# url-kaist/UV-SLAM

Hardware: AMD Instinct MI355X
Metric: sliding-window solves/sec (10 KF, 150 pts, 40 lines, 3 VP) (higher is better)
Workload: dtype f64; 1 GPU; W10-P150-L40-V3 x 256 independent windows per GPU (BASELINE configs[2]); single window (configs[1]) in single_window, the 20k-point window (configs[3]) in large_window (both with --full); windows_per_gpu=256, frames=11, points=150, lines=40, vp_tagged_lines=30, prior=True, parallelism=replicas x1

## Files before the change

### uv-slam_amd/csrc/uvs_solve_kernel.h

```cpp
#pragma once
#include <hip/hip_runtime.h>
#include <initializer_list>
#include <utility>
#include "../../include/uvs_solver.h"
#include "uvs_layout.h"
#include "uvs_factors.h"

namespace uvsdev {

#ifndef UVS_UNIT
#define UVS_UNIT unit
#endif

#ifndef UVS_X_PLAIN_TID
static __device__ __forceinline__ int lane_tid() { int t = threadIdx.x; asm volatile("" : "+v"(t)); return t; }
#else
static __device__ __forceinline__ int lane_tid() { return threadIdx.x; }
#endif
static constexpr int NT = UVS_NT;
static constexpr int NW = NT / 64;
static constexpr bool ROLES = NT > 256;
static constexpr int ET = ROLES ? 256 : NT;
static constexpr int EW = ET / 64;
static constexpr int GT0 = NT - UVS_GT;
// ... 14 lines not shown
static_assert(UVS_PT_C == UVS_PT_A + 12, "pt_anchor_pass reads A and c as one run");
static constexpr int CP_PB = NT > 256 ? UVS_T_CP_PB : 4;
static constexpr int CP_LB = NT > 256 ? UVS_T_CP_LB : 2;
static constexpr int BS_LNB = NT > 256 ? UVS_T_BS_LNB : 4;
static constexpr int PR_UN = NT > 256 ? UVS_T_PR_UN : 26;
static constexpr int PG_UN = NT > 256 ? 16 : 32;

static constexpr int L_X = 0;
static constexpr int L_XC = L_X + UVS_XDIM;
static constexpr int L_G = L_XC + UVS_XDIM;
static constexpr int L_DLT = L_G + UVS_RD;
static constexpr int L_HD = L_DLT + UVS_RD + 24;
static constexpr int L_SC = L_HD + UVS_RD;
static constexpr int L_DD = L_SC + UVS_RD;
static constexpr int L_DINV = L_DD + UVS_RD;
static constexpr int L_RF = L_DINV + UVS_RD;
static constexpr int L_EX = L_RF + 120;
static constexpr int L_PDX = L_EX + 16;
static constexpr int L_PR = L_PDX + UVS_MAX_PRIOR_DIM;
static constexpr int L_PRC = L_PR + UVS_MAX_PRIOR_DIM;
static constexpr int L_RED = L_PRC + UVS_MAX_PRIOR_DIM;
static constexpr int L_CTRL = L_RED + (5 * NW > 24 ? 5 * NW : 24);
static constexpr int L_PROF = L_CTRL + 32;
static constexpr int L_WPROF = L_PROF + 24;
static constexpr int L_LCOST = L_WPROF + 8;
static constexpr int LACC = 1;
static constexpr int L_LGMAX = L_LCOST + ET / LACC;
static constexpr int L_PX0 = L_LGMAX + 8;
static constexpr int L_PTAB = L_PX0 + 9 * UVS_MAX_PRIOR_BLOCKS;
static constexpr int L_SMALL = (L_PTAB + 2 * UVS_MAX_PRIOR_BLOCKS + 1) & ~1;
static constexpr int L_S = L_SMALL;
static constexpr int L_TOTAL = L_S + UVS_S_DOUBLES;
static_assert(L_TOTAL * 8 <= 160 * 1024, "LDS map exceeds the 160 KB of a CU");
enum { P_SETUP = 0, P_OBS, P_LMPREP, P_GATHER, P_ASSEMBLE, P_CHOL, P_TRSV, P_BACKSUB, P_COST, P_MISC, P_CH_DIAG, P_CH_PANEL, P_CH_TRAIL, P_AS_IMU, P_AS_ZERO, P_AS_ADD, P_LAST };
#define UVS_PROF(c, k) do { if ((c).o.debug && lane_tid() == 0) { const long long now_ = clock64(); (c).sh[L_PROF + (k)] += (double)(now_ - (long long)(c).sh[L_PROF + 23]); (c).sh[L_PROF + 23] = (double)now_; } } while (0)
static constexpr size_t LDS_BYTES = (size_t)L_TOTAL * 8;
static constexpr int TL_PER_WAVE = 4096;
inline namespace UVS_UNIT { __device__ long long g_lin_tl[8 * TL_PER_WAVE * 2]; }
#define UVS_TLOG(c, id) do { if ((c).o.debug == 5 && (threadIdx.x & 63) == 0 && blockIdx.x == 0) { const int w_ = threadIdx.x >> 6; const int n_ = (int)(c).sh[L_WPROF + w_]; \
    if (n_ < TL_PER_WAVE) { g_lin_tl[2 * (w_ * TL_PER_WAVE + n_)] = (id); g_lin_tl[2 * (w_ * TL_PER_WAVE + n_) + 1] = clock64(); (c).sh[L_WPROF + w_] = (double)(n_ + 1); } } } while (0)

enum { C_COST = 0, C_RADIUS, C_DECR, C_XNORM, C_GMAX, C_CAND, C_MCC, C_STEP2, C_XC2, C_GO, C_IT, C_INVALID, C_CUR, C_FIRST,
       C_TERM, C_NSUCC, C_CHOLOK, C_GMAXLM, C_TIMEUP };

struct KOpts {
    int max_it, ex_free, keep_cand, jacobi;
    double sqrt_info, line_factor, vp_factor, loss_pt, loss_ln, loss_vp, G[3];
    double r0, rmax, rmin, min_rel, dlo, dhi, ftol, gtol, ptol;
    int max_invalid;
    int debug;
    long long max_ticks;
    int redamp;
    int line_ahead;
};

inline namespace UVS_UNIT {
__constant__ unsigned char c_blk_fa[UVS_NBLK];
__constant__ unsigned char c_blk_fb[UVS_NBLK];
}

UVS_DEV int sidx(int i, int j) {
    const int bi = i >> 4, bj = j >> 4;
    return (((bi * (bi + 1)) >> 1) + bj) * UVS_BLK_SZ + (i & 15) * UVS_BLK_LD + (j & 15);
}
UVS_DEV double bcast_lane(double v, int lane) {
    const int lo = __builtin_amdgcn_readlane(__double2loint(v), lane);
    const int hi = __builtin_amdgcn_readlane(__double2hiint(v), lane);
    return __hiloint2double(hi, lo);
}
UVS_DEV void wave_sync() {
    __builtin_amdgcn_fence(__ATOMIC_RELEASE, "wavefront");
    __builtin_amdgcn_wave_barrier();
    __builtin_amdgcn_fence(__ATOMIC_ACQUIRE, "wavefront");
}

UVS_DEV double wave_sum(double v) {
#pragma unroll
    for (int off = 32; off > 0; off >>= 1) v += __shfl_down(v, off, 64);
    return v;
}
UVS_DEV double wave_max(double v) {
#pragma unroll
    for (int off = 32; off > 0; off >>= 1) v = fmax(v, __shfl_down(v, off, 64));
    return v;
}
UVS_DEV void rsqrt_pair(double x, double* sq, double* rsq) {
    const double y = __builtin_amdgcn_rsq(x);
    double g = x * y, hh = 0.5 * y;
    double r = fma(-hh, g, 0.5);
    g = fma(g, r, g); hh = fma(hh, r, hh);
    r = fma(-hh, g, 0.5);
    g = fma(g, r, g); hh = fma(hh, r, hh);
    const double d = fma(-g, g, x);
    g = fma(d, hh, g);
    *sq = g; *rsq = 2.0 * hh;
}
UVS_DEV void block_reduce(double* sh, double* s , double* mx) {
    const int tid = lane_tid(), lane = tid & 63, wv = tid >> 6;
    __syncthreads();
#pragma unroll
    for (int k = 0; k < 4; ++k) { const double t = wave_sum(s[k]); if (lane == 0) sh[L_RED + wv * 5 + k] = t; }
    { const double t = wave_max(*mx); if (lane == 0) sh[L_RED + wv * 5 + 4] = t; }
    __syncthreads();
    double a[4] = {0, 0, 0, 0}, m = 0.0;
#pragma unroll
    for (int w = 0; w < NW; ++w) {
// ... 1123 lines not shown
    UVS_TLOG(c, 43);
}
UVS_DEV double lin_imu_tiles(const Ctx& c, ImuN& N) {
    DevWinK& h = *c.hdr;
    double* sh = c.sh;
    const int tid = lane_tid(), lane = tid & 63, wv = UVS_KWAVE(tid), li = lane & 15, lk = lane >> 4;
    double cost = 0.0;
    double* IM = sh + L_S;
    IntK* itab = (IntK*)c.bi + h.i_imu;
    bool act[IMU_SLOTS];
#pragma unroll
    for (int s = 0; s < IMU_SLOTS; ++s) {
        const int b = imu_block_of(wv, s);
        act[s] = b < h.n_imu && !itab[2 * (b < h.n_imu ? b : 0) + 1];
        N.act[s] = act[s]; N.fi[s] = itab[2 * (b < h.n_imu ? b : 0)];
        if (act[s]) {
            double* Jb = IM + IMU_BLK * b; const double* Wb = Jb + IMU_WOFF;
            d4_t t0 = {0.0, 0.0, 0.0, 0.0}, t1 = t0;
            double wa[4], j0[4], j1[4];
#pragma unroll
            for (int q = 0; q < 4; ++q) { wa[q] = Wb[li * UVS_BLK_LD + 4 * q + lk]; j0[q] = Jb[(4 * q + lk) * IMU_JLD + li]; j1[q] = Jb[(4 * q + lk) * IMU_JLD + 16 + li]; }
#pragma unroll
            for (int q = 0; q < 4; ++q) { t0 = __builtin_amdgcn_mfma_f64_16x16x4f64(wa[q], j0[q], t0, 0, 0, 0); t1 = __builtin_amdgcn_mfma_f64_16x16x4f64(wa[q], j1[q], t1, 0, 0, 0); }
#pragma unroll
            for (int q = 0; q < 4; ++q) { Jb[(lk + 4 * q) * IMU_JLD + li] = t0[q]; Jb[(lk + 4 * q) * IMU_JLD + 16 + li] = t1[q]; }
        }
    }
    wave_sync();
#pragma unroll
    for (int s = 0; s < IMU_SLOTS; ++s) {
        const int b = imu_block_of(wv, s);
        d4_t n00 = {0.0, 0.0, 0.0, 0.0}, n10 = n00, n11 = n00;
        if (act[s]) {
            const double* Jb = IM + IMU_BLK * b;
            double j0[4], j1[4];
#pragma unroll
            for (int q = 0; q < 4; ++q) { j0[q] = Jb[(4 * q + lk) * IMU_JLD + li]; j1[q] = Jb[(4 * q + lk) * IMU_JLD + 16 + li]; }
#pragma unroll
            for (int q = 0; q < 4; ++q) {
                n00 = __builtin_amdgcn_mfma_f64_16x16x4f64(j0[q], j0[q], n00, 0, 0, 0);
                n10 = __builtin_amdgcn_mfma_f64_16x16x4f64(j1[q], j0[q], n10, 0, 0, 0);
                n11 = __builtin_amdgcn_mfma_f64_16x16x4f64(j1[q], j1[q], n11, 0, 0, 0);
            }
            if (lane == 63) cost += 0.5 * n11[3];
        }
        N.n00[s] = n00; N.n10[s] = n10; N.n11[s] = n11;
    }
    UVS_PROF(c, P_AS_IMU);
    return cost;
}
UVS_DEV double lin_imu(const Ctx& c, const double* x, ImuN& N) { lin_imu_stage(c, x); return lin_imu_tiles(c, N); }
UVS_DEV double lin_frames(const Ctx& c, const double* x, ImuN& N) { const double pc = lin_prep(c, x); return pc + lin_imu(c, x, N); }

UVS_DEV void spd4_inverse(const double* H, const double* gl, double* X, double* hg) {
    double L[10];
    double i0, i1, i2, i3;
    rsqrt_pair(H[0], &L[0], &i0);
    L[1] = H[1] * i0; rsqrt_pair(H[2] - L[1] * L[1], &L[2], &i1);
    L[3] = H[3] * i0; L[4] = (H[4] - L[3] * L[1]) * i1; rsqrt_pair(H[5] - L[3] * L[3] - L[4] * L[4], &L[5], &i2);
    L[6] = H[6] * i0; L[7] = (H[7] - L[6] * L[1]) * i1; L[8] = (H[8] - L[6] * L[3] - L[7] * L[4]) * i2;
    rsqrt_pair(H[9] - L[6] * L[6] - L[7] * L[7] - L[8] * L[8], &L[9], &i3);
    hg[0] = 0.0; hg[1] = 0.0; hg[2] = 0.0; hg[3] = 0.0;
#pragma unroll
    for (int cidx = 0; cidx < 4; ++cidx) {
        double e[4] = {0, 0, 0, 0}; e[cidx] = 1.0;
        e[0] = e[0] * i0;
        e[1] = (e[1] - L[1] * e[0]) * i1;
        e[2] = (e[2] - L[3] * e[0] - L[4] * e[1]) * i2;
        e[3] = (e[3] - L[6] * e[0] - L[7] * e[1] - L[8] * e[2]) * i3;
        e[3] = e[3] * i3;
        e[2] = (e[2] - L[8] * e[3]) * i2;
        e[1] = (e[1] - L[4] * e[2] - L[7] * e[3]) * i1;
        e[0] = (e[0] - L[1] * e[1] - L[3] * e[2] - L[6] * e[3]) * i0;
        X[0 * 4 + cidx] = e[0]; X[1 * 4 + cidx] = e[1]; X[2 * 4 + cidx] = e[2]; X[3 * 4 + cidx] = e[3];
#pragma unroll
        for (int a = 0; a < 4; ++a) hg[a] += e[a] * gl[cidx];
    }
}

#ifndef UVS_X_NO_LISTS_BY_GATHERERS
static constexpr bool LISTS_BY_GATHERERS = ROLES;
#else
static constexpr bool LISTS_BY_GATHERERS = false;
#endif
struct ChunkDesc { int type, k0, k1, o0, nob, nlm, nlist; const int* glists; };
UVS_DEV ChunkDesc chunk_desc(const Ctx& c, int ch) {
    DevWinK& h = *c.hdr;
    IntK* chunks = (IntK*)c.bi + h.i_chunks + UVS_CHUNK_INTS * UVS_KIDX(ch);
    ChunkDesc d;
    d.type = chunks[0]; d.k0 = chunks[1]; d.k1 = chunks[2];
    d.glists = c.bi + h.i_lists + chunks[3];
    d.nlist = chunks[4];
    d.nlm = d.k1 - d.k0;
    d.o0 = chunks[6]; d.nob = chunks[7];
    return d;
}
UVS_DEV int* chunk_lists(const Ctx& c, const ChunkDesc& d) {
    DevWinK& h = *c.hdr;
    double* rec = c.sh + L_S;
    if (d.type == 0) return (int*)(rec + (size_t)d.nob * h.pt_rec + (size_t)(d.nob + h.pt_xslots * d.nlm) * 12);
    return (int*)(rec + (size_t)d.nob * (UVS_LN_REC + 2 * UVS_LN_EY) + 20 * d.nlm);
}
UVS_DEV void pt_landmark_slots(const Ctx& c, const ChunkDesc& d, int k, int b0, int b1, double hd, double gl, double dd, double hinv, double ginv, double* gmax_lm) {
    DevWinK& h = *c.hdr;
    const int PREC = h.pt_rec, XS = h.pt_xslots, li = k - d.k0;
    double* rec = c.sh + L_S;
    double* Eb = rec + (size_t)d.nob * PREC;
    double* EIb = Eb + (size_t)(d.nob + XS * d.nlm) * 6;
    double* E = Eb + (size_t)(b0 + XS * li) * 6; double* EI = EIb + (size_t)(b0 + XS * li) * 6;
    double* Eg = c.ws + h.w_pt_E + 6 * (size_t)(d.o0 + b0 + XS * k);
        double* px = c.ws + h.w_pt_x + 4 * (size_t)k; px[0] = ginv; px[1] = gl; px[2] = dd; px[3] = hd;
        *gmax_lm = fmax(*gmax_lm, fabs(gl));
        double e0[6] = {0, 0, 0, 0, 0, 0}, etd = 0.0;
        for (int o = b0; o < b1; ++o) {
            const double* Ro = rec + (size_t)o * PREC;
#pragma unroll
            for (int a = 0; a < 6; ++a) e0[a] += Ro[UVS_PT_C] * Ro[UVS_PT_A + a] + Ro[UVS_PT_C + 1] * Ro[UVS_PT_A + 6 + a];
            if (h.td_on) etd += Ro[UVS_PT_C] * Ro[UVS_PT_TD] + Ro[UVS_PT_C + 1] * Ro[UVS_PT_TD + 1];
        }
#pragma unroll
        for (int a = 0; a < 6; ++a) { E[a] = e0[a]; EI[a] = e0[a] * hinv; Eg[a] = e0[a] * hinv; }
        if (h.td_on) {
            const int st_ = 6 * (b1 - b0 + 1);
#pragma unroll
            for (int a = 0; a < 6; ++a) { const double e = a == 0 ? etd : 0.0; E[st_ + a] = e; EI[st_ + a] = e * hinv; Eg[st_ + a] = e * hinv; }
        }
        if (h.ex_on) {
            double ex6[6] = {0, 0, 0, 0, 0, 0};
            for (int o = b0; o < b1; ++o) {
                const double* Ro = rec + (size_t)o * PREC;
// ... 79 lines not shown
        double* Eb = c.sh + L_S + (size_t)d.nob * PREC;
        double* E = Eb + (size_t)(b0 + li) * 6; double* EI = E + (size_t)(d.nob + d.nlm) * 6;
#pragma unroll
        for (int a = 0; a < 6; ++a) { E[a] = e0[a]; EI[a] = e0[a] * hinv; Eg[a] = e0[a] * hinv; }
    }
    lacc_add(c.sh, 0.0, gmax_lm);
}
UVS_DEV void chunk_touch(const Ctx& c, const ChunkDesc& d, const double* invd, const double* line) {
    DevWinK& h = *c.hdr;
    const int tid = lane_tid();
    if (tid >= d.nob) return;
    const int o = d.o0 + tid;
    double acc = 0.0; int iacc = 0;
    if (d.type == 0) {
        const int lm = c.bi[h.i_pt_lm + o]; iacc = c.bi[h.i_pt_fi + o] + c.bi[h.i_pt_fj + o];
        const double* m = c.bd + h.d_ptmeas + o; const int st = h.pt_stride;
#pragma unroll
        for (int q = 0; q < 6; ++q) acc += m[q * st];
        acc += invd[lm] + c.ws[h.w_scale_pt + lm];
        iacc += c.bi[h.i_pt_beg + lm] + c.bi[h.i_pt_beg + lm + 1];
    } else {
        const int lm = c.bi[h.i_ln_lm + o]; iacc = c.bi[h.i_ln_fj + o] + c.bi[h.i_ln_vp + o];
#ifndef UVS_X_NO_TOUCH_B1
        iacc += c.bi[h.i_ln_beg + lm] + c.bi[h.i_ln_beg + lm + 1];
        acc += c.ws[h.w_scale_ln + 4 * lm] + c.ws[h.w_scale_ln + 4 * lm + 3];
#endif
        const double* m = c.bd + h.d_lnmeas + o; const int st = h.ln_stride;
#pragma unroll
        for (int q = 0; q < 9; ++q) acc += m[q * st];
        const double* ltrig = line_trig_of(c, line);
        if (ltrig) {
#pragma unroll
            for (int q = 0; q < 8; ++q) acc += ltrig[8 * lm + q];
        } else {
#pragma unroll
            for (int q = 0; q < 4; ++q) acc += line[4 * lm + q];
        }
    }
    asm volatile("" :: "v"(acc), "v"(iacc));
}
static constexpr int LG_UN = 16;
UVS_DEV void copy_lists_gatherers(const Ctx& c, const ChunkDesc& d) {
    int* lists = chunk_lists(c, d);
    const int t0 = lane_tid() - GT0;
    for (int tb = t0; tb < d.nlist; tb += LG_UN * UVS_GT) {
        int w[LG_UN];
#pragma unroll
        for (int u = 0; u < LG_UN; ++u) { const int t = tb + u * UVS_GT; w[u] = d.glists[t < d.nlist ? t : tb]; }
#pragma unroll
        for (int u = 0; u < LG_UN; ++u) { const int t = tb + u * UVS_GT; if (t < d.nlist) lists[t] = w[u]; }
    }
}
UVS_DEV double line_pass_a(const Ctx& c, const ChunkDesc& d, const double* x, const double* line, int rec_base);
UVS_DEV void line_pass_b(const Ctx& c, const ChunkDesc& d, bool first, double radius, double cost, int rec_base);
UVS_DEV void chunk_eval(const Ctx& c, const ChunkDesc& d, const double* x, const double* invd, const double* line, bool first, double radius) {
    DevWinK& h = *c.hdr;
    double* sh = c.sh;
    const int tid = lane_tid();
    const double* RF = sh + L_RF; const double* ric = sh + L_EX; const double* tic = sh + L_EX + 9;
    double cost = 0.0, gmax_lm = 0.0;
    {
        const int type = d.type, k0 = d.k0, k1 = d.k1;
        const int* glists = d.glists;
        const int nlist = d.nlist;
        const int nlm = d.nlm;
        UVS_TLOG(c, 1);
        __syncthreads();
        UVS_PROF(c, P_GATHER);
        UVS_TLOG(c, 2);
        if (type == 0) {
            const int* beg = c.bi + h.i_pt_beg;
            const int o0 = d.o0, nob = d.nob, o1 = o0 + nob;
            const int PREC = h.pt_rec, XS = h.pt_xslots;
            double* rec = sh + L_S;
            double* Eb = rec + (size_t)nob * PREC;
            double* EIb = Eb + (size_t)(nob + XS * nlm) * 6;
            int* lists = (int*)(EIb + (size_t)(nob + XS * nlm) * 6);
            if (!LISTS_BY_GATHERERS) for (int t = tid; t < nlist; t += ET) lists[t] = glists[t];
            for (int o = o0 + tid; o < o1; o += ET) {
                const int lm = c.bi[h.i_pt_lm + o], fi = c.bi[h.i_pt_fi + o], fj = c.bi[h.i_pt_fj + o];
                double pi[3], pj[3], vij[4] = {0.0, 0.0, 0.0, 0.0};
                load_point_obs(c, o, x[183], pi, pj, vij);
                double r[2], A[12], B[12], cl[2], jtd[2] = {0.0, 0.0};
                point_eval<true, false>(x + 7 * fi, RF + 9 * fi, pose_of(x, fj), RF + 9 * fj, ric, tic, invd[lm], pi, pj, c.o.sqrt_info, r, A, B, cl, nullptr,
                                        vij, vij + 2, h.td_on ? jtd : nullptr);
                double sc; cost += 0.5 * cauchy(c.o.loss_pt, r[0] * r[0] + r[1] * r[1], &sc);
                double* R = rec + (size_t)(o - o0) * PREC;
                R[0] = sc * r[0]; R[1] = sc * r[1];
#pragma unroll
                for (int q = 0; q < 12; ++q) { R[UVS_PT_A + q] = sc * A[q]; R[UVS_PT_B + q] = sc * B[q]; }
                R[UVS_PT_C] = sc * cl[0]; R[UVS_PT_C + 1] = sc * cl[1];
                if (h.td_on || h.ex_on) { R[UVS_PT_TD] = sc * jtd[0]; R[UVS_PT_TD + 1] = sc * jtd[1]; R[UVS_PT_TD + 2] = 0.0; R[UVS_PT_TD + 3] = 0.0; }
                if (h.ex_on) {
                    double r2[2], A2[12], B2[12], cl2[2], jex[12];
                    point_eval<true, true>(x + 7 * fi, RF + 9 * fi, pose_of(x, fj), RF + 9 * fj, ric, tic, invd[lm], pi, pj, c.o.sqrt_info, r2, A2, B2, cl2, jex);
#pragma unroll
                    for (int q = 0; q < 12; ++q) R[UVS_PT_EX + q] = sc * jex[q];
                }
            }
            UVS_TLOG(c, 3);
            __syncthreads();
            UVS_PROF(c, P_OBS);
            UVS_TLOG(c, 4);
            for (int ol = tid; ol < nob; ol += ET) {
                const int k = c.bi[h.i_pt_lm + o0 + ol], li = k - k0, b0 = beg[k] - o0, b1 = beg[k + 1] - o0;
                double hd, gl; pt_landmark_hd_gl(rec, PREC, b0, b1, &hd, &gl);
                const bool lead = ol == b0;
                double sc;
                if (first) { sc = c.o.jacobi ? 1.0 / (1.0 + sqrt(hd)) : 1.0; if (lead && !ANCHOR_BY_GATHERERS) c.ws[h.w_scale_pt + k] = sc; } else sc = c.ws[h.w_scale_pt + k];
                const double dd = fmin(fmax(sc * sc * hd, c.o.dlo), c.o.dhi) / (radius * sc * sc);
                const double hinv = 1.0 / (hd + dd), ginv = gl * hinv;
                const int s = ol - b0 + 1;
                double* E = Eb + (size_t)(b0 + XS * li) * 6; double* EI = EIb + (size_t)(b0 + XS * li) * 6;
                double* Eg = c.ws + h.w_pt_E + 6 * (size_t)(o0 + b0 + XS * k);
                double* R = rec + (size_t)ol * PREC;
                const double c0 = R[UVS_PT_C], c1 = R[UVS_PT_C + 1], rr0 = R[0], rr1 = R[1];
                double Bv[12];
#pragma unroll
                for (int a = 0; a < 12; ++a) Bv[a] = R[UVS_PT_B + a];
#pragma unroll
                for (int a = 0; a < 6; ++a) { const double e = c0 * Bv[a] + c1 * Bv[6 + a]; E[6 * s + a] = e; EI[6 * s + a] = e * hinv; Eg[6 * s + a] = e * hinv; }
                R[UVS_PT_RC2] = rr0 - c0 * ginv; R[UVS_PT_RC2 + 1] = rr1 - c1 * ginv;
                if (lead && !ANCHOR_BY_GATHERERS) pt_landmark_slots(c, d, k, b0, b1, hd, gl, dd, hinv, ginv, &gmax_lm);
            }
            UVS_TLOG(c, 5);
            __syncthreads();
            UVS_PROF(c, P_LMPREP);
            UVS_TLOG(c, 7);
            lacc_add(sh, cost, gmax_lm);
        } else {
            if (!LISTS_BY_GATHERERS) { int* lists = chunk_lists(c, d); for (int t = tid; t < nlist; t += ET) lists[t] = glists[t]; }
            cost = line_pass_a(c, d, x, line, 0);
            UVS_TLOG(c, 3);
            __syncthreads();
            UVS_PROF(c, P_OBS);
            UVS_TLOG(c, 4);
            line_pass_b(c, d, first, radius, cost, 0);
        }
    }
}
UVS_DEV double line_pass_a(const Ctx& c, const ChunkDesc& d, const double* x, const double* line, int rec_base) {
    DevWinK& h = *c.hdr;
    const int tid = lane_tid();
    const double* RF = c.sh + L_RF; const double* ric = c.sh + L_EX; const double* tic = c.sh + L_EX + 9;
    double cost = 0.0;
    {
        {
            const int k0 = d.k0, o0 = d.o0, o1 = o0 + d.nob;
            double* rec = c.sh + L_S + rec_base;
            const double* ltrig = line_trig_of(c, line);
            for (int o = o0 + tid; o < o1; o += ET) {
                const int lm = c.bi[h.i_ln_lm + o], fj = c.bi[h.i_ln_fj + o], hv = c.bi[h.i_ln_vp + o];
                const double* m = c.bd + h.d_lnmeas + o; const int st = h.ln_stride;
                const double sp[3] = {m[0], m[st], m[2 * st]}, ep[3] = {m[3 * st], m[4 * st], m[5 * st]}, vp[3] = {m[6 * st], m[7 * st], m[8 * st]};
                LineGeom g;
                line_geom<true>(x + 7 * fj, x + 7 * fj + 3, RF + 9 * fj, ric, tic, line + 4 * lm, g, ltrig ? ltrig + 8 * lm : nullptr);
                double* R = rec + (size_t)(o - o0) * UVS_LN_REC;
                double r[2], Jp[12], Jl[8], sc;
                line_residual<true>(g, sp, ep, c.o.line_factor, r, Jp, Jl);
                cost += 0.5 * cauchy(c.o.loss_ln, r[0] * r[0] + r[1] * r[1], &sc);
                R[0] = sc * r[0]; R[1] = sc * r[1];
#pragma unroll
                for (int q = 0; q < 12; ++q) R[UVS_LN_JP + q] = sc * Jp[q];
#pragma unroll
                for (int q = 0; q < 8; ++q) R[UVS_LN_JL + q] = sc * Jl[q];
                R[UVS_LN_RV + 1] = (double)((lm - k0) | (fj << 10));
                if (hv) {
                    double rv, Jvp[6], Jvl[4];
                    vp_residual<true>(g, vp, c.o.vp_factor, &rv, Jvp, Jvl);
                    cost += 0.5 * cauchy(c.o.loss_vp, rv * rv, &sc);
                    R[UVS_LN_RV] = sc * rv;
#pragma unroll
                    for (int q = 0; q < 6; ++q) R[UVS_LN_JP + 12 + q] = sc * Jvp[q];
#pragma unroll
                    for (int q = 0; q < 4; ++q) R[UVS_LN_JL + 8 + q] = sc * Jvl[q];
                } else {
#pragma unroll
                    for (int q = 0; q < 6; ++q) R[UVS_LN_JP + 12 + q] = 0.0;
                    R[UVS_LN_RV] = 0.0;
#pragma unroll
                    for (int q = 0; q < 4; ++q) R[UVS_LN_JL + 8 + q] = 0.0;
                }
            }
        }
    }
    return cost;
}
UVS_DEV void line_pass_b(const Ctx& c, const ChunkDesc& d, bool first, double radius, double cost, int rec_base) {
    DevWinK& h = *c.hdr;
    double* sh = c.sh;
    const int tid = lane_tid();
    double gmax_lm = 0.0;
    {
        {
            const int* beg = c.bi + h.i_ln_beg;
            const int k0 = d.k0, nlm = d.nlm, o0 = d.o0, nob = d.nob;
            double* rec = sh + L_S + rec_base;
            double* Eb = sh + L_S + (size_t)nob * UVS_LN_REC;
            double* Yb = Eb + (size_t)nob * UVS_LN_EY;
            double* Xb = Yb + (size_t)nob * UVS_LN_EY;
            for (int li = tid; li < nlm; li += ET) {
                const int k = k0 + li, b0 = beg[k] - o0, b1 = beg[k + 1] - o0;
                double H[10] = {0, 0, 0, 0, 0, 0, 0, 0, 0, 0}, gl[4] = {0, 0, 0, 0};
                double scl[4] = {1.0, 1.0, 1.0, 1.0};
                if (!first) {
#pragma unroll
                    for (int a = 0; a < 4; ++a) scl[a] = c.ws[h.w_scale_ln + 4 * k + a];
                }
                for (int o = b0; o < b1; ++o) {
                    const double* R = rec + (size_t)o * UVS_LN_REC;
#pragma unroll
                    for (int a = 0; a < 4; ++a) {
                        gl[a] += R[UVS_LN_JL + a] * R[0] + R[UVS_LN_JL + 4 + a] * R[1] + R[UVS_LN_JL + 8 + a] * R[UVS_LN_RV];
#pragma unroll
                        for (int b = 0; b <= a; ++b) H[(a * (a + 1)) / 2 + b] += R[UVS_LN_JL + a] * R[UVS_LN_JL + b] + R[UVS_LN_JL + 4 + a] * R[UVS_LN_JL + 4 + b] + R[UVS_LN_JL + 8 + a] * R[UVS_LN_JL + 8 + b];
                    }
                }
                double* lx = c.ws + h.w_ln_x + UVS_LN_X * (size_t)k;
#pragma unroll
                for (int q = 0; q < 10; ++q) lx[12 + q] = H[q];
#pragma unroll
                for (int a = 0; a < 4; ++a) {
                    const double hd = H[(a * (a + 1)) / 2 + a];
                    double sc;
                    if (first) { sc = c.o.jacobi ? 1.0 / (1.0 + sqrt(hd)) : 1.0; c.ws[h.w_scale_ln + 4 * k + a] = sc; } else sc = scl[a];
                    const double dd = fmin(fmax(sc * sc * hd, c.o.dlo), c.o.dhi) / (radius * sc * sc);
                    H[(a * (a + 1)) / 2 + a] = hd + dd;
                    lx[4 + a] = gl[a]; lx[8 + a] = dd;
                    gmax_lm = fmax(gmax_lm, fabs(gl[a]));
                }
                double* X = Xb + 20 * li;
                double hg[4];
                spd4_inverse(H, gl, X, hg);
#pragma unroll
                for (int a = 0; a < 4; ++a) { X[16 + a] = hg[a]; lx[a] = hg[a]; }
            }
            UVS_TLOG(c, 5);
            __syncthreads();
            UVS_TLOG(c, 6);
            for (int o = tid; o < nob; o += ET) {
                double* R = rec + (size_t)o * UVS_LN_REC;
                const int li = (int)R[UVS_LN_RV + 1] & 1023;
                double* E = Eb + (size_t)o * UVS_LN_EY; double* Y = Yb + (size_t)o * UVS_LN_EY;
                double* Yg = c.ws + h.w_ln_Y + 24 * (size_t)(o0 + o);
                double Xv[20], Jl[12], Jp[18];
#pragma unroll
                for (int q = 0; q < 20; ++q) Xv[q] = Xb[20 * li + q];
#pragma unroll
                for (int q = 0; q < 12; ++q) Jl[q] = R[UVS_LN_JL + q];
#pragma unroll
                for (int q = 0; q < 18; ++q) Jp[q] = R[UVS_LN_JP + q];
                const double rr0 = R[0], rr1 = R[1], rr2 = R[UVS_LN_RV];
#pragma unroll
                for (int a = 0; a < 6; ++a) {
                    double e[4];
#pragma unroll
                    for (int q = 0; q < 4; ++q) { e[q] = Jl[q] * Jp[a] + Jl[4 + q] * Jp[6 + a] + Jl[8 + q] * Jp[12 + a]; E[6 * q + a] = e[q]; }
#pragma unroll
                    for (int q = 0; q < 4; ++q) { const double y = Xv[4 * q] * e[0] + Xv[4 * q + 1] * e[1] + Xv[4 * q + 2] * e[2] + Xv[4 * q + 3] * e[3]; Y[6 * q + a] = y; Yg[6 * q + a] = y; }
                }
                R[0] = rr0 - (Jl[0] * Xv[16] + Jl[1] * Xv[17] + Jl[2] * Xv[18] + Jl[3] * Xv[19]);
                R[1] = rr1 - (Jl[4] * Xv[16] + Jl[5] * Xv[17] + Jl[6] * Xv[18] + Jl[7] * Xv[19]);
                R[UVS_LN_RV] = rr2 - (Jl[8] * Xv[16] + Jl[9] * Xv[17] + Jl[10] * Xv[18] + Jl[11] * Xv[19]);
            }
            __syncthreads();
            UVS_PROF(c, P_LMPREP);
            UVS_TLOG(c, 7);
            lacc_add(sh, cost, gmax_lm);
        }
    }
}
UVS_DEV int chunk_eval_barriers(const ChunkDesc& d) { return d.type == 0 ? 3 : 4; }
UVS_DEV void chunk_gather(const Ctx& c, const ChunkDesc& d, int grp, GAcc& acc, int rec_base = 0) {
    DevWinK& h = *c.hdr;
    const double* rec = c.sh + L_S;
    const int* lists = chunk_lists(c, d);
    UVS_TLOG(c, 8);
    if (d.type == 0) {
        const long long tg0_ = clock64();
// ... 15 lines not shown
    double* sh = c.sh;
    const int tid = lane_tid();
    const int type = d.type, k0 = d.k0;
    const int* glists = d.glists;
    const int nlist = d.nlist;
    const int nlm = d.nlm;
    __syncthreads();
    double* rec = sh + L_S;
    if (type == 0) {
        const int* beg = c.bi + h.i_pt_beg;
        const int o0 = d.o0, nob = d.nob;
        const int PREC = h.pt_rec, XS = h.pt_xslots;
        double* Gb = rec;
        double* Eb = rec + (size_t)nob * PREC;
        double* EIb = Eb + (size_t)(nob + XS * nlm) * 6;
        int* lists = (int*)(EIb + (size_t)(nob + XS * nlm) * 6);
        for (int t = tid; t < nlist; t += ET) lists[t] = glists[t];
        for (int t = tid; t < nlm + nob; t += ET) {
            const bool anchor = t < nlm;
            const int ol = anchor ? 0 : t - nlm;
            const int k = anchor ? k0 + t : c.bi[h.i_pt_lm + o0 + ol], li = k - k0;
            const int nobs = beg[k + 1] - beg[k];
            if (nobs == 0) continue;
            double* px = c.ws + h.w_pt_x + 4 * (size_t)k;
            const double gl = px[1], dd_old = px[2], hd = px[3], sc = c.ws[h.w_scale_pt + k];
            const double dd = fmin(fmax(sc * sc * hd, c.o.dlo), c.o.dhi) / (radius * sc * sc);
            const double hdo = hd + dd_old, hinv = 1.0 / (hd + dd), dh = hinv - 1.0 / hdo;
            const int slot = anchor ? (beg[k] - o0) + XS * li : ol + XS * li + 1;
            double* Eg = c.ws + h.w_pt_E + 6 * (size_t)(anchor ? beg[k] + XS * k : o0 + ol + XS * k + 1);
            double e[6];
#pragma unroll
            for (int a = 0; a < 6; ++a) e[a] = Eg[a] * hdo;
#pragma unroll
            for (int a = 0; a < 6; ++a) { Eb[6 * slot + a] = e[a]; EIb[6 * slot + a] = e[a] * dh; Gb[6 * slot + a] = e[a] * dh * gl; Eg[a] = e[a] * hinv; }
        }
        __syncthreads();
        for (int li = tid; li < nlm; li += ET) {
            const int k = k0 + li;
            if (beg[k + 1] == beg[k]) continue;
            double* px = c.ws + h.w_pt_x + 4 * (size_t)k;
            const double gl = px[1], hd = px[3], sc = c.ws[h.w_scale_pt + k];
            const double dd = fmin(fmax(sc * sc * hd, c.o.dlo), c.o.dhi) / (radius * sc * sc);
            px[0] = gl * (1.0 / (hd + dd)); px[2] = dd;
        }
    } else {
        const int o0 = d.o0, nob = d.nob;
        double* T = rec;
        double* Gb = rec + (size_t)nlm * 34;
        double* Eb = rec + (size_t)nob * UVS_LN_REC;
        double* Yb = Eb + (size_t)nob * UVS_LN_EY;
        double* Xb = Yb + (size_t)nob * UVS_LN_EY;
        int* lists = (int*)(Xb + 20 * nlm);
        for (int t = tid; t < nlist; t += ET) lists[t] = glists[t];
        for (int li = tid; li < nlm; li += ET) {
            const int k = k0 + li;
            double* lx = c.ws + h.w_ln_x + UVS_LN_X * (size_t)k;
            double H[10], gl[4], ddo[4], hgo[4], hg[4];
#pragma unroll
            for (int q = 0; q < 10; ++q) H[q] = lx[12 + q];
#pragma unroll
            for (int a = 0; a < 4; ++a) { hgo[a] = lx[a]; gl[a] = lx[4 + a]; ddo[a] = lx[8 + a]; }
            double* t = T + 34 * li;
#pragma unroll
            for (int q = 0; q < 10; ++q) t[20 + q] = H[q];
#pragma unroll
            for (int a = 0; a < 4; ++a) {
                const double hd = H[(a * (a + 1)) / 2 + a], sc = c.ws[h.w_scale_ln + 4 * k + a];
                const double dd = fmin(fmax(sc * sc * hd, c.o.dlo), c.o.dhi) / (radius * sc * sc);
                H[(a * (a + 1)) / 2 + a] = hd + dd;
                t[30 + a] = ddo[a]; lx[8 + a] = dd;
            }
            spd4_inverse(H, gl, t, hg);
#pragma unroll
            for (int a = 0; a < 4; ++a) { t[16 + a] = hg[a] - hgo[a]; lx[a] = hg[a]; }
        }
        __syncthreads();
        for (int o = tid; o < nob; o += ET) {
            const int li = c.bi[h.i_ln_lm + o0 + o] - k0;
            double tv[34], yo[24];
#pragma unroll
            for (int q = 0; q < 34; ++q) tv[q] = T[34 * li + q];
            double* Yg = c.ws + h.w_ln_Y + 24 * (size_t)(o0 + o);
#pragma unroll
            for (int q = 0; q < 24; ++q) yo[q] = Yg[q];
            double* E = Eb + (size_t)o * UVS_LN_EY; double* Y = Yb + (size_t)o * UVS_LN_EY; double* G = Gb + (size_t)o * 6;
#pragma unroll
            for (int a = 0; a < 6; ++a) {
                double e[4];
#pragma unroll
                for (int q = 0; q < 4; ++q) {
                    double v = tv[30 + q] * yo[6 * q + a];
#pragma unroll
                    for (int p2 = 0; p2 < 4; ++p2) { const int hi_ = q > p2 ? q : p2, lo_ = q > p2 ? p2 : q; v += tv[20 + (hi_ * (hi_ + 1)) / 2 + lo_] * yo[6 * p2 + a]; }
                    e[q] = v; E[6 * q + a] = v;
                }
                double ga = 0.0;
#pragma unroll
                for (int q = 0; q < 4; ++q) {
                    const double yn = tv[4 * q] * e[0] + tv[4 * q + 1] * e[1] + tv[4 * q + 2] * e[2] + tv[4 * q + 3] * e[3];
                    Y[6 * q + a] = yn - yo[6 * q + a]; Yg[6 * q + a] = yn;
                    ga += e[q] * tv[16 + q];
                }
                G[a] = ga;
            }
        }
        __syncthreads();
    }
}
UVS_DEV void redamp_gather(const Ctx& c, const ChunkDesc& d, int grp, GAcc& acc) {
    const double* rec = c.sh + L_S;
    const int* lists = chunk_lists(c, d);
    if (d.type == 0) gather_points<false, true>(grp, lists, rec, acc, -d.nob * c.hdr->pt_rec);
    else gather_lines<true>(grp, lists, rec, acc, d.nlm * 34, d.nob * UVS_LN_REC);
}
UVS_DEV void redamp_chunk(const Ctx& c, int ch, double radius, int grp, GAcc& acc) {
    const ChunkDesc d = chunk_desc(c, ch);
    redamp_prep(c, d, radius);
    redamp_gather(c, d, grp, acc);
}
static constexpr int R2_R = 0, R2_RR = 1056, R2_G = 1092, R2_HD = 1098, R2_SC = 1104, R2_DD = 1110, R2_MI = 1116, R2_MG = 1152, R2_Z = 1158, R2_DR = 2214;
static_assert(R2_DR + 6 <= UVS_RELO2_DOUBLES, "side buffer");
// ... 337 lines not shown
    if (mode != 2) asm_prior(c);
    __syncthreads();
    UVS_PROF(c, P_AS_ADD);
    if (mode == 1) return;
    asm_finish(c, x, first, radius, cost, gmax_lm, mode);
    UVS_PROF(c, P_ASSEMBLE);
}

static constexpr int ROLE_PARTS_OFF = (UVS_NF - 1) * IMU_BLK;
static_assert(ROLE_PARTS_OFF + (8 * GR + 1) * UVS_GT <= UVS_S_DOUBLES, "IMU staging + part sums exceed the S region");
UVS_DEV void role_barriers(int n) { for (int i = 0; i < n; ++i) __syncthreads(); }
UVS_DEV void gacc_store(const Ctx& c, const GAcc& A) {
    double* W = c.ws + c.hdr->w_gacc + (lane_tid() - GT0);
#pragma unroll
    for (int q = 0; q < 6 * GR; ++q) __builtin_nontemporal_store(A.v[q], W + q * UVS_GT);
#pragma unroll
    for (int q = 0; q < GR; ++q) { __builtin_nontemporal_store(A.g[q], W + (6 * GR + q) * UVS_GT); __builtin_nontemporal_store(A.hd[q], W + (7 * GR + q) * UVS_GT); }
}
UVS_DEV void gacc_load(const Ctx& c, GAcc& A) {
    const double* W = c.ws + c.hdr->w_gacc + (lane_tid() - GT0);
#pragma unroll
    for (int q = 0; q < 6 * GR; ++q) A.v[q] = W[q * UVS_GT];
#pragma unroll
    for (int q = 0; q < GR; ++q) { A.g[q] = W[(6 * GR + q) * UVS_GT]; A.hd[q] = W[(7 * GR + q) * UVS_GT]; }
}
#ifndef UVS_X_NO_LINE_AHEAD
static constexpr bool LINE_AHEAD = ROLES;
#else
static constexpr bool LINE_AHEAD = false;
#endif
static constexpr int DBG_N_LIN = 21, DBG_N_AHEAD = 22;
UVS_DEV int line_ahead_base(const Ctx& c, const ChunkDesc& d, int rb, const ChunkDesc& dn) {
    if (!LINE_AHEAD || !c.o.line_ahead || dn.type != 1) return -1;
    DevWinK& h = *c.hdr;
    const int rsz = d.nob * (d.type == 0 ? h.pt_rec : UVS_LN_REC);
    return uvs_line_ahead_base(uvs_chunk_end(d.type, d.nob, d.nlm, d.nlist, h.pt_rec, h.pt_xslots), rb, rsz, dn.type, dn.nob, dn.nlm, dn.nlist);
}
UVS_DEV void linearize_roles(const Ctx& c, const double* x, const double* invd, const double* line, bool first, double radius, int prep_mode, bool redamp) {
    DevWinK& h = *c.hdr;
    const bool ev = role_eval();
    { const double pc = lin_prep(c, x, redamp ? 2 : prep_mode); if (!redamp) lacc_set(c.sh, pc, 0.0); }
    double ic = 0.0;
    UVS_TLOG(c, 20);
    PriorAdd pa;
    ImuN N;
    if (ev) {
        ChunkDesc d = chunk_desc(c, 0);
        int rb = -1;
        double acost = 0.0;
        for (int ch = 0; ch < h.n_chunks; ++ch) {
            if (redamp) redamp_prep(c, d, radius);
            else if (rb >= 0) {
                UVS_TLOG(c, 1);
                __syncthreads();
                UVS_PROF(c, P_GATHER);
                UVS_TLOG(c, 2);
                line_pass_b(c, d, first, radius, acost, rb);
                __syncthreads();
            } else {
                chunk_eval(c, d, x, invd, line, first, radius);
            }
            if (ch + 1 < h.n_chunks) {
                const ChunkDesc dn = chunk_desc(c, ch + 1);
                rb = redamp ? -1 : line_ahead_base(c, d, rb > 0 ? rb : 0, dn);
                d = dn;
                if (rb >= 0) {
                    UVS_TLOG(c, 9);
                    acost = line_pass_a(c, d, x, line, rb);
                    UVS_TLOG(c, 3);
                    if (c.o.debug && lane_tid() == 0) c.sh[L_PROF + DBG_N_AHEAD] += 1.0;
                }
#ifdef UVS_CHUNK_TOUCH
                else if (!redamp) chunk_touch(c, d, invd, line);
#endif
            }
        }
        UVS_TLOG(c, 21);
        lin_imu_stage(c, x);
#ifndef UVS_X_NO_PRIOR_AHEAD
        asm_prior_load(c, pa);
#endif
        ic = lin_imu_tiles(c, N);
        UVS_TLOG(c, 22);
        __syncthreads();
        asm_zero(c);
        __syncthreads();
        UVS_TLOG(c, 23);
        __syncthreads();
        UVS_TLOG(c, 24);
        asm_imu(c, N);
        UVS_TLOG(c, 25);
    } else {
        const int grp = gather_group(c);
        GAcc A;
        if (redamp) gacc_load(c, A); else gacc_zero(A);
        ChunkDesc d = chunk_desc(c, 0);
        int rb = 0;
        for (int ch = 0; ch < h.n_chunks; ++ch) {
            if (redamp) { role_barriers(redamp_barriers(d)); redamp_gather(c, d, grp, A); }
            else {
                __syncthreads();
                if (LISTS_BY_GATHERERS) copy_lists_gatherers(c, d);
                AnchorPre ap; ap.b0 = 0; ap.b1 = 0; ap.sc = 1.0;
                if (ANCHOR_BY_GATHERERS && d.type == 0) pt_anchor_pre(c, d, first, ap);
                __syncthreads();
                if (ANCHOR_BY_GATHERERS && d.type == 0) pt_anchor_pass(c, d, first, radius, ap);
                role_barriers(chunk_eval_barriers(d) - 2);
                chunk_gather(c, d, grp, A, rb);
            }
            if (ch + 1 < h.n_chunks) {
// ... 610 lines not shown
```

### uv-slam_amd/csrc/uvs_solver_handle.h

```cpp
#pragma once
#include <algorithm>
#include <chrono>
#include <condition_variable>
#include <cstdlib>
#include <functional>
#include <memory>
#include <mutex>
#include <pthread.h>
#include <sched.h>
#include <string>
#include <thread>
#include <vector>

#include "../../include/uvs_solver.h"
#include "uvs_hip_buf.h"
#include "uvs_layout.h"
#include "uvs_pack.h"
#include "uvs_solve_kernel.h"

#pragma GCC visibility push(hidden)

struct PackPool {
    std::vector<std::thread> th; std::mutex m; std::condition_variable cv_go, cv_done;
    const std::function<void(int)>* job = nullptr; int gen = 0, pending = 0; bool stop = false;
// ... 70 lines not shown
    std::vector<long long> blob_off, ws_off;
    std::vector<char> host_blobs;
    std::unique_ptr<MargDevScratch> marg_dev;
    std::unique_ptr<MargBatchBuf> marg_batch;
    std::unique_ptr<MargWorker> marg_worker;
    uvs_prior marg_job_out;
    std::unique_ptr<uvspack::PackCache> pack_cache;
    std::vector<std::vector<char>> slot_blobs;
    std::shared_ptr<PackPool> pool;
    DevBuf<char> d_blobs;
    PinnedBuf<char> h_up;
    DevBuf<double> d_ws;
    long long* d_blob_off = nullptr; long long* d_ws_off = nullptr;
    std::vector<long long> out_tab; long long* d_out_tab = nullptr; DevBuf<double> d_outpack; long long out_total = 0;
    PinnedBuf<char> h_out;
    DevBuf<uvs_report> d_reports;
    DevBuf<double> d_dbg;
    uvsdev::EvalScratch eval_scratch;
    struct Large {
        bool active = false; int n_chunks = 0, sel = 0, it = 0, invalid = 0, nsucc = 0, pending = 0, term = 0, status = 0;
        bool need_lin = true, first = true, done = false;
        bool stored = false; int backsub_wgs = 0;
        double radius = 0, decr = 2, cost = 0, gmax = 0, x_norm = 0, local_x2 = 0;
        uvs_report rep;
        double frame_x2 = 0;
        double relo_pose_in[7] = {0, 0, 0, 0, 0, 0, 0};
        int grid = 0;
        std::chrono::steady_clock::time_point t_begin;
    } L;
    struct LargeBufs {
        DevBuf<double> d_state, d_partials, d_reduced, d_bsums, d_out, d_sc5;
        DevBuf<double> d_ctl; DevBuf<uvs_report> d_rep;
        DevBuf<double> d_fimg;
        void* comm = nullptr; int rank = 0, nranks = 1;
        int step_nranks = 1;
        bool debug_step = false; DevBuf<double> d_lstep;
    } LB;
    uvs_solver(); ~uvs_solver();
};

inline uvsdev::KOpts make_kopts(const uvs_options& o, int debug) {
    uvsdev::KOpts k;
    k.max_it = o.max_num_iterations; k.ex_free = o.estimate_extrinsic; k.keep_cand = o.function_tol_keeps_candidate; k.jacobi = o.jacobi_scaling;
    k.sqrt_info = o.point_sqrt_info; k.line_factor = o.line_factor; k.vp_factor = o.vp_factor;
    k.loss_pt = o.loss_point; k.loss_ln = o.loss_line; k.loss_vp = o.loss_vp;
    k.G[0] = o.gravity[0]; k.G[1] = o.gravity[1]; k.G[2] = o.gravity[2];
    k.r0 = o.initial_trust_region_radius; k.rmax = o.max_trust_region_radius; k.rmin = o.min_trust_region_radius;
    k.min_rel = o.min_relative_decrease; k.dlo = o.min_lm_diagonal; k.dhi = o.max_lm_diagonal;
    k.ftol = o.function_tolerance; k.gtol = o.gradient_tolerance; k.ptol = o.parameter_tolerance;
    k.max_ticks = o.max_solver_time_in_seconds > 0.0 ? std::max(1LL, (long long)(o.max_solver_time_in_seconds * 1e8)) : 0LL;
    k.max_invalid = o.max_consecutive_invalid_steps; k.debug = debug;
    { const char* e = std::getenv("UVS_REDAMP"); k.redamp = (e && e[0] == '0') ? 0 : 1; }
    { const char* e = std::getenv("UVS_LINE_AHEAD"); k.line_ahead = (e && e[0] == '0') ? 0 : 1; }
    return k;
}

inline PackPool& pack_pool(uvs_solver* s) { if (!s->pool) s->pool = std::make_shared<PackPool>(); return *s->pool; }

int upload_windows(uvs_solver* s, int n, const uvs_window* const* ws, bool wait, int chunk_grid = 0, bool out_direct = false, bool all_blocks = false);
int marg_unit_init(const unsigned char* fa, const unsigned char* fb, int n);
void marg_worker_release(uvs_solver* s);
int large_unit_init(const unsigned char* fa, const unsigned char* fb, int n);
int debug_step_large(uvs_solver* s, const uvs_window* w, int n_radii, const double* radii, int n_step, double* step, double* scal);
#pragma GCC visibility pop
```

Measured before the change: 195,300 solves/s.

## Spread per-line 4x4 normal-equation build and solve across eight lanes

Line pass B and the redamp path used to give each line to one thread, which accumulated the full 4x4 Hessian and gradient and then did a Cholesky solve. Now eight lanes share a line: each lane accumulates one or two Hessian/gradient entries, the entries are gathered with DPP quad moves, and every lane factors redundantly and solves one inverse column. Line offsets and scales are also preloaded before the barrier. This buys more parallelism and shorter serial chains per line, at the cost of redundant factorization, cross-lane moves, and a new env flag that is on by default.

```diff
diff --git a/uv-slam_amd/csrc/uvs_solve_kernel.h b/uv-slam_amd/csrc/uvs_solve_kernel.h
--- a/uv-slam_amd/csrc/uvs_solve_kernel.h
+++ b/uv-slam_amd/csrc/uvs_solve_kernel.h
@@ -90,6 +90,7 @@
     long long max_ticks;
     int redamp;
     int line_ahead;
+    int line_b1;
 };
 
 inline namespace UVS_UNIT {
@@ -1319,30 +1320,84 @@
 UVS_DEV double lin_imu(const Ctx& c, const double* x, ImuN& N) { lin_imu_stage(c, x); return lin_imu_tiles(c, N); }
 UVS_DEV double lin_frames(const Ctx& c, const double* x, ImuN& N) { const double pc = lin_prep(c, x); return pc + lin_imu(c, x, N); }
 
+UVS_DEV void spd4_factor(const double* H, double* L, double* inv) {
+    rsqrt_pair(H[0], &L[0], &inv[0]);
+    L[1] = H[1] * inv[0]; rsqrt_pair(H[2] - L[1] * L[1], &L[2], &inv[1]);
+    L[3] = H[3] * inv[0]; L[4] = (H[4] - L[3] * L[1]) * inv[1]; rsqrt_pair(H[5] - L[3] * L[3] - L[4] * L[4], &L[5], &inv[2]);
+    L[6] = H[6] * inv[0]; L[7] = (H[7] - L[6] * L[1]) * inv[1]; L[8] = (H[8] - L[6] * L[3] - L[7] * L[4]) * inv[2];
+    rsqrt_pair(H[9] - L[6] * L[6] - L[7] * L[7] - L[8] * L[8], &L[9], &inv[3]);
+}
+UVS_DEV void spd4_column(const double* L, const double* inv, int cidx, double* e) {
+#pragma unroll
+    for (int q = 0; q < 4; ++q) e[q] = q == cidx ? 1.0 : 0.0;
+    e[0] = e[0] * inv[0];
+    e[1] = (e[1] - L[1] * e[0]) * inv[1];
+    e[2] = (e[2] - L[3] * e[0] - L[4] * e[1]) * inv[2];
+    e[3] = (e[3] - L[6] * e[0] - L[7] * e[1] - L[8] * e[2]) * inv[3];
+    e[3] = e[3] * inv[3];
+    e[2] = (e[2] - L[8] * e[3]) * inv[2];
+    e[1] = (e[1] - L[4] * e[2] - L[7] * e[3]) * inv[1];
+    e[0] = (e[0] - L[1] * e[1] - L[3] * e[2] - L[6] * e[3]) * inv[0];
+}
 UVS_DEV void spd4_inverse(const double* H, const double* gl, double* X, double* hg) {
-    double L[10];
-    double i0, i1, i2, i3;
-    rsqrt_pair(H[0], &L[0], &i0);
-    L[1] = H[1] * i0; rsqrt_pair(H[2] - L[1] * L[1], &L[2], &i1);
-    L[3] = H[3] * i0; L[4] = (H[4] - L[3] * L[1]) * i1; rsqrt_pair(H[5] - L[3] * L[3] - L[4] * L[4], &L[5], &i2);
-    L[6] = H[6] * i0; L[7] = (H[7] - L[6] * L[1]) * i1; L[8] = (H[8] - L[6] * L[3] - L[7] * L[4]) * i2;
-    rsqrt_pair(H[9] - L[6] * L[6] - L[7] * L[7] - L[8] * L[8], &L[9], &i3);
+    double L[10], inv[4];
+    spd4_factor(H, L, inv);
     hg[0] = 0.0; hg[1] = 0.0; hg[2] = 0.0; hg[3] = 0.0;
 #pragma unroll
     for (int cidx = 0; cidx < 4; ++cidx) {
-        double e[4] = {0, 0, 0, 0}; e[cidx] = 1.0;
-        e[0] = e[0] * i0;
-        e[1] = (e[1] - L[1] * e[0]) * i1;
-        e[2] = (e[2] - L[3] * e[0] - L[4] * e[1]) * i2;
-        e[3] = (e[3] - L[6] * e[0] - L[7] * e[1] - L[8] * e[2]) * i3;
-        e[3] = e[3] * i3;
-        e[2] = (e[2] - L[8] * e[3]) * i2;
-        e[1] = (e[1] - L[4] * e[2] - L[7] * e[3]) * i1;
-        e[0] = (e[0] - L[1] * e[1] - L[3] * e[2] - L[6] * e[3]) * i0;
+        double e[4];
+        spd4_column(L, inv, cidx, e);
         X[0 * 4 + cidx] = e[0]; X[1 * 4 + cidx] = e[1]; X[2 * 4 + cidx] = e[2]; X[3 * 4 + cidx] = e[3];
 #pragma unroll
         for (int a = 0; a < 4; ++a) hg[a] += e[a] * gl[cidx];
     }
+}
+#ifndef UVS_X_B1_ONE_LANE
+static constexpr bool LINE_B1_LANES = true;
+#else
+static constexpr bool LINE_B1_LANES = false;
+#endif
+static constexpr int LB1_G = 8;
+static constexpr int LB1_TRIP = ET / LB1_G;
+static_assert(64 % LB1_G == 0, "the lanes of a line sit in one wave");
+UVS_DEV double ln_term3(double x0, double y0, double x1, double y1, double x2, double y2) { return fma(x2, y2, fma(x0, y0, x1 * y1)); }
+UVS_DEV double ln_damping(const KOpts& o, double sc, double hd, double radius) { return fmin(fmax(sc * sc * hd, o.dlo), o.dhi) / (radius * sc * sc); }
+template <int CTRL> UVS_DEV double dpp_move(double v) {
+    const int lo = __builtin_amdgcn_update_dpp(0, __double2loint(v), CTRL, 0xf, 0xf, true);
+    const int hi = __builtin_amdgcn_update_dpp(0, __double2hiint(v), CTRL, 0xf, 0xf, true);
+    return __hiloint2double(hi, lo);
+}
+template <int C> UVS_DEV double quad_lane(double v) { return dpp_move<C * 0x55>(v); }
+UVS_DEV double upper_quad(double v) { return dpp_move<0x104>(v); }
+static_assert(LB1_G == 8, "a line's group is two quads of one row of 16 lanes");
+template <int C> UVS_DEV void ln_hg_stage(const double* e, double glc, double* hg) {
+#pragma unroll
+    for (int a = 0; a < 4; ++a) hg[a] = quad_lane<C>(hg[a] + e[a] * glc);
+}
+struct LnLane { int j, q0, q1, a1, b1; };
+UVS_DEV LnLane ln_lane(int tid) {
+    LnLane l; l.j = tid & (LB1_G - 1);
+    l.q0 = (l.j * (l.j + 3)) >> 1;
+    l.a1 = l.j < 1 ? 1 : l.j < 3 ? 2 : 3; l.b1 = l.j < 6 ? l.j - ((l.a1 * (l.a1 - 1)) >> 1) : 0;
+    l.q1 = ((l.a1 * (l.a1 + 1)) >> 1) + l.b1;
+    return l;
+}
+UVS_DEV void ln_lanes_solve(const KOpts& o, int j, double s0, double s1, double sc, double radius, double* dd, double* e, double* hg) {
+    *dd = ln_damping(o, sc, s0, radius);
+    const double d0 = j < 4 ? s0 + *dd : s0;
+    const double u0 = upper_quad(d0), u1 = upper_quad(s1);
+    double H[10], gl[4];
+    H[0] = quad_lane<0>(d0); H[2] = quad_lane<1>(d0); H[5] = quad_lane<2>(d0); H[9] = quad_lane<3>(d0);
+    gl[0] = quad_lane<0>(u0); gl[1] = quad_lane<1>(u0); gl[2] = quad_lane<2>(u0); gl[3] = quad_lane<3>(u0);
+    H[1] = quad_lane<0>(s1); H[3] = quad_lane<1>(s1); H[4] = quad_lane<2>(s1); H[6] = quad_lane<3>(s1);
+    H[7] = quad_lane<0>(u1); H[8] = quad_lane<1>(u1);
+    double L[10], inv[4];
+    spd4_factor(H, L, inv);
+    spd4_column(L, inv, j & 3, e);
+    hg[0] = 0.0; hg[1] = 0.0; hg[2] = 0.0; hg[3] = 0.0;
+    ln_hg_stage<0>(e, gl[0], hg); ln_hg_stage<1>(e, gl[1], hg); ln_hg_stage<2>(e, gl[2], hg);
+#pragma unroll
+    for (int a = 0; a < 4; ++a) hg[a] += e[a] * gl[3];
 }
 
 #ifndef UVS_X_NO_LISTS_BY_GATHERERS
@@ -1528,7 +1583,20 @@
     }
 }
 UVS_DEV double line_pass_a(const Ctx& c, const ChunkDesc& d, const double* x, const double* line, int rec_base);
-UVS_DEV void line_pass_b(const Ctx& c, const ChunkDesc& d, bool first, double radius, double cost, int rec_base);
+struct LnB1Pre { int b0, b1; double sc; };
+UVS_DEV LnB1Pre line_b1_preload(const Ctx& c, const ChunkDesc& d, bool first) {
+    LnB1Pre p; p.b0 = 0; p.b1 = 0; p.sc = 1.0;
+    if (LINE_B1_LANES && c.o.line_b1 && d.nlm > 0) {
+        DevWinK& h = *c.hdr;
+        const int tid = lane_tid(), li = tid / LB1_G;
+        const int k = d.k0 + (li < d.nlm ? li : d.nlm - 1);
+        const int* beg = c.bi + h.i_ln_beg;
+        p.b0 = beg[k] - d.o0; p.b1 = beg[k + 1] - d.o0;
+        if (!first) p.sc = c.ws[h.w_scale_ln + 4 * k + (tid & 3)];
+    }
+    return p;
+}
+UVS_DEV void line_pass_b(const Ctx& c, const ChunkDesc& d, bool first, double radius, double cost, int rec_base, const LnB1Pre& pre);
 UVS_DEV void chunk_eval(const Ctx& c, const ChunkDesc& d, const double* x, const double* invd, const double* line, bool first, double radius) {
     DevWinK& h = *c.hdr;
     double* sh = c.sh;
@@ -1608,10 +1676,11 @@
             if (!LISTS_BY_GATHERERS) { int* lists = chunk_lists(c, d); for (int t = tid; t < nlist; t += ET) lists[t] = glists[t]; }
             cost = line_pass_a(c, d, x, line, 0);
             UVS_TLOG(c, 3);
+            const LnB1Pre pre = line_b1_preload(c, d, first);
             __syncthreads();
             UVS_PROF(c, P_OBS);
             UVS_TLOG(c, 4);
-            line_pass_b(c, d, first, radius, cost, 0);
+            line_pass_b(c, d, first, radius, cost, 0, pre);
         }
     }
 }
@@ -1662,7 +1731,7 @@
     }
     return cost;
 }
-UVS_DEV void line_pass_b(const Ctx& c, const ChunkDesc& d, bool first, double radius, double cost, int rec_base) {
+UVS_DEV void line_pass_b(const Ctx& c, const ChunkDesc& d, bool first, double radius, double cost, int rec_base, const LnB1Pre& pre) {
     DevWinK& h = *c.hdr;
     double* sh = c.sh;
     const int tid = lane_tid();
@@ -1675,6 +1744,54 @@
             double* Eb = sh + L_S + (size_t)nob * UVS_LN_REC;
             double* Yb = Eb + (size_t)nob * UVS_LN_EY;
             double* Xb = Yb + (size_t)nob * UVS_LN_EY;
+            if (LINE_B1_LANES && c.o.line_b1) {
+                const LnLane l = ln_lane(tid);
+                const int j = l.j;
+                const int x0 = UVS_LN_JL + (j & 3), y0 = j < 4 ? x0 : 0, y01 = j < 4 ? x0 + 4 : 1, y02 = j < 4 ? x0 + 8 : UVS_LN_RV;
+                const int x1 = UVS_LN_JL + l.a1, y1 = UVS_LN_JL + l.b1;
+                for (int l0 = 0; l0 < nlm; l0 += LB1_TRIP) {
+                    const int li = l0 + tid / LB1_G;
+                    const bool on = li < nlm;
+                    const int k = k0 + (on ? li : nlm - 1);
+                    int b0 = pre.b0, b1 = pre.b1;
+                    double sc = pre.sc;
+                    if (l0 > 0) {
+                        b0 = beg[k] - o0; b1 = beg[k + 1] - o0;
+                        if (!first) sc = c.ws[h.w_scale_ln + 4 * k + (j & 3)];
+                    }
+                    double s0 = 0.0, s1 = 0.0;
+                    {
+                        const double* R = rec + (size_t)b0 * UVS_LN_REC;
+                        const double *px0 = R + x0, *py0 = R + y0, *py01 = R + y01, *py02 = R + y02, *px1 = R + x1, *py1 = R + y1;
+                        for (int n = b1 - b0; n > 0; --n) {
+                            s0 += ln_term3(px0[0], py0[0], px0[4], py01[0], px0[8], py02[0]);
+                            s1 += ln_term3(px1[0], py1[0], px1[4], py1[4], px1[8], py1[8]);
+                            px0 += UVS_LN_REC; py0 += UVS_LN_REC; py01 += UVS_LN_REC; py02 += UVS_LN_REC; px1 += UVS_LN_REC; py1 += UVS_LN_REC;
+                        }
+                    }
+                    if (first) sc = c.o.jacobi ? 1.0 / (1.0 + sqrt(s0)) : 1.0;
+                    double dd, e[4], hg[4];
+                    ln_lanes_solve(c.o, j, s0, s1, sc, radius, &dd, e, hg);
+                    double* lx = c.ws + h.w_ln_x + UVS_LN_X * (size_t)k;
+                    gmax_lm = fmax(gmax_lm, j < 4 ? 0.0 : fabs(s0));
+                    if (on) {
+                        lx[j < 4 ? 12 + l.q0 : j] = s0;
+                        lx[12 + l.q1] = s1;
+                        if (j < 4) {
+                            double* X = Xb + 20 * li;
+#pragma unroll
+                            for (int q = 0; q < 4; ++q) X[4 * q + j] = e[q];
+                            lx[8 + j] = dd;
+                            if (first) c.ws[h.w_scale_ln + 4 * k + j] = sc;
+                        }
+                        if (j == 3) {
+                            double* X = Xb + 20 * li;
+#pragma unroll
+                            for (int a = 0; a < 4; ++a) { X[16 + a] = hg[a]; lx[a] = hg[a]; }
+                        }
+                    }
+                }
+            } else
             for (int li = tid; li < nlm; li += ET) {
                 const int k = k0 + li, b0 = beg[k] - o0, b1 = beg[k + 1] - o0;
                 double H[10] = {0, 0, 0, 0, 0, 0, 0, 0, 0, 0}, gl[4] = {0, 0, 0, 0};
@@ -1687,9 +1804,9 @@
                     const double* R = rec + (size_t)o * UVS_LN_REC;
 #pragma unroll
                     for (int a = 0; a < 4; ++a) {
-                        gl[a] += R[UVS_LN_JL + a] * R[0] + R[UVS_LN_JL + 4 + a] * R[1] + R[UVS_LN_JL + 8 + a] * R[UVS_LN_RV];
-#pragma unroll
-                        for (int b = 0; b <= a; ++b) H[(a * (a + 1)) / 2 + b] += R[UVS_LN_JL + a] * R[UVS_LN_JL + b] + R[UVS_LN_JL + 4 + a] * R[UVS_LN_JL + 4 + b] + R[UVS_LN_JL + 8 + a] * R[UVS_LN_JL + 8 + b];
+                        gl[a] += ln_term3(R[UVS_LN_JL + a], R[0], R[UVS_LN_JL + 4 + a], R[1], R[UVS_LN_JL + 8 + a], R[UVS_LN_RV]);
+#pragma unroll
+                        for (int b = 0; b <= a; ++b) H[(a * (a + 1)) / 2 + b] += ln_term3(R[UVS_LN_JL + a], R[UVS_LN_JL + b], R[UVS_LN_JL + 4 + a], R[UVS_LN_JL + 4 + b], R[UVS_LN_JL + 8 + a], R[UVS_LN_JL + 8 + b]);
                     }
                 }
                 double* lx = c.ws + h.w_ln_x + UVS_LN_X * (size_t)k;
@@ -1700,7 +1817,7 @@
                     const double hd = H[(a * (a + 1)) / 2 + a];
                     double sc;
                     if (first) { sc = c.o.jacobi ? 1.0 / (1.0 + sqrt(hd)) : 1.0; c.ws[h.w_scale_ln + 4 * k + a] = sc; } else sc = scl[a];
-                    const double dd = fmin(fmax(sc * sc * hd, c.o.dlo), c.o.dhi) / (radius * sc * sc);
+                    const double dd = ln_damping(c.o, sc, hd, radius);
                     H[(a * (a + 1)) / 2 + a] = hd + dd;
                     lx[4 + a] = gl[a]; lx[8 + a] = dd;
                     gmax_lm = fmax(gmax_lm, fabs(gl[a]));
@@ -1822,6 +1939,37 @@
         double* Xb = Yb + (size_t)nob * UVS_LN_EY;
         int* lists = (int*)(Xb + 20 * nlm);
         for (int t = tid; t < nlist; t += ET) lists[t] = glists[t];
+        if (LINE_B1_LANES && c.o.line_b1) {
+            const LnLane l = ln_lane(tid);
+            const int j = l.j;
+            for (int l0 = 0; l0 < nlm; l0 += LB1_TRIP) {
+                const int li = l0 + tid / LB1_G;
+                const bool on = li < nlm;
+                const int k = k0 + (on ? li : nlm - 1);
+                double* lx = c.ws + h.w_ln_x + UVS_LN_X * (size_t)k;
+                double* t = T + 34 * li;
+                const double s0 = lx[j < 4 ? 12 + l.q0 : j];
+                const double s1 = lx[12 + l.q1];
+                const double sc = c.ws[h.w_scale_ln + 4 * k + (j & 3)], ddo = lx[8 + (j & 3)];
+                double hgo[4];
+#pragma unroll
+                for (int a = 0; a < 4; ++a) hgo[a] = lx[a];
+                double dd, e[4], hg[4];
+                ln_lanes_solve(c.o, j, s0, s1, sc, radius, &dd, e, hg);
+                if (on) {
+                    if (j < 6) t[20 + l.q1] = s1;
+                    if (j < 4) {
+                        t[20 + l.q0] = s0; t[30 + j] = ddo; lx[8 + j] = dd;
+#pragma unroll
+                        for (int q = 0; q < 4; ++q) t[4 * q + j] = e[q];
+                    }
+                    if (j == 3) {
+#pragma unroll
+                        for (int a = 0; a < 4; ++a) { t[16 + a] = hg[a] - hgo[a]; lx[a] = hg[a]; }
+                    }
+                }
+            }
+        } else
         for (int li = tid; li < nlm; li += ET) {
             const int k = k0 + li;
             double* lx = c.ws + h.w_ln_x + UVS_LN_X * (size_t)k;
@@ -1836,7 +1984,7 @@
 #pragma unroll
             for (int a = 0; a < 4; ++a) {
                 const double hd = H[(a * (a + 1)) / 2 + a], sc = c.ws[h.w_scale_ln + 4 * k + a];
-                const double dd = fmin(fmax(sc * sc * hd, c.o.dlo), c.o.dhi) / (radius * sc * sc);
+                const double dd = ln_damping(c.o, sc, hd, radius);
                 H[(a * (a + 1)) / 2 + a] = hd + dd;
                 t[30 + a] = ddo[a]; lx[8 + a] = dd;
             }
@@ -2280,10 +2428,11 @@
             if (redamp) redamp_prep(c, d, radius);
             else if (rb >= 0) {
                 UVS_TLOG(c, 1);
+                const LnB1Pre pre = line_b1_preload(c, d, first);
                 __syncthreads();
                 UVS_PROF(c, P_GATHER);
                 UVS_TLOG(c, 2);
-                line_pass_b(c, d, first, radius, acost, rb);
+                line_pass_b(c, d, first, radius, acost, rb, pre);
                 __syncthreads();
             } else {
                 chunk_eval(c, d, x, invd, line, first, radius);
diff --git a/uv-slam_amd/csrc/uvs_solver_handle.h b/uv-slam_amd/csrc/uvs_solver_handle.h
--- a/uv-slam_amd/csrc/uvs_solver_handle.h
+++ b/uv-slam_amd/csrc/uvs_solver_handle.h
@@ -146,6 +146,7 @@
     k.max_invalid = o.max_consecutive_invalid_steps; k.debug = debug;
     { const char* e = std::getenv("UVS_REDAMP"); k.redamp = (e && e[0] == '0') ? 0 : 1; }
     { const char* e = std::getenv("UVS_LINE_AHEAD"); k.line_ahead = (e && e[0] == '0') ? 0 : 1; }
+    { const char* e = std::getenv("UVS_LINE_B1"); k.line_b1 = (e && e[0] == '0') ? 0 : 1; }
     return k;
 }
 
```

After: 198,200 solves/s, median of 6. 1.02x the previous value.
